# pyannote/pyannote-audio

Hardware: AMD Instinct MI355X
Metric: audio-hours/sec (real-time factor) for speaker-diarization-3.1 pipeline (higher is better)
Workload: dtype f32

## Files before the change

### include/pyannote_amd.h

```cpp
#ifndef PYANNOTE_AMD_H
#define PYANNOTE_AMD_H

#include <stddef.h>
#include <stdint.h>

#ifdef __cplusplus
extern "C" {
#endif

int pa_version(void);
const char* pa_last_error(void);

void pa_prof_enable(int on);
size_t pa_prof_report(char* buf, size_t cap);

#define PA_MAX_LSTM_LAYERS 8
#define PA_MAX_LINEAR 4

typedef struct pa_seg_weights {
  int32_t sinc_stride;
  int32_t lstm_layers;
  int32_t lstm_hidden;
  int32_t lstm_bidir;
  int32_t num_linear;
// ... 75 lines not shown
  int32_t num_blocks[4];
  int32_t planes[4];
  int32_t bottleneck;
  const float* fb_window;
  const float* fb_tw256;
  const float* fb_tw512;
  const float* fb_mel_w;
  const int32_t* fb_mel_lo;
  const int32_t* fb_mel_hi;
  const float* stem_w;
  const float* stem_shift;
  const float* blk_w1[PA_MAX_RES_BLOCKS];
  const float* blk_shift1[PA_MAX_RES_BLOCKS];
  const float* blk_w2[PA_MAX_RES_BLOCKS];
  const float* blk_shift2[PA_MAX_RES_BLOCKS];
  const float* blk_u1[PA_MAX_RES_BLOCKS];
  const float* blk_u2[PA_MAX_RES_BLOCKS];
  const float* blk_wsc[PA_MAX_RES_BLOCKS];
  const float* blk_shiftsc[PA_MAX_RES_BLOCKS];
  const float* blk_w3[PA_MAX_RES_BLOCKS];
  const float* blk_shift3[PA_MAX_RES_BLOCKS];
  const float* seg1_w;
  const float* seg1_b;
  const float* blk_v1[PA_MAX_RES_BLOCKS];
  const float* blk_v2[PA_MAX_RES_BLOCKS];
  int32_t fb_center_kernel;
} pa_emb_weights;

int pa_emb_num_fbank_frames(int num_samples);
int pa_emb_num_pool_frames(const pa_emb_weights* w, int num_samples);
size_t pa_emb_workspace_bytes(const pa_emb_weights* w, int num_chunks, int num_samples, int num_masks);
int pa_emb_forward(const pa_emb_weights* w, const float* wav, int64_t wav_len, int64_t chunk_stride,
                   int num_chunks, int num_samples, const float* masks, int num_masks, int mask_frames,
                   const int32_t* nearest_idx, float* emb, void* workspace, size_t workspace_bytes,
                   void* stream);

size_t pa_emb_ragged_workspace_bytes(const pa_emb_weights* w, int num_utterances, int max_samples);
int pa_emb_forward_ragged(const pa_emb_weights* w, const float* wav, int64_t wav_len, const int64_t* offsets,
                          const int32_t* lengths, int num_utterances, int max_samples, const float* masks, float* emb,
                          void* workspace, size_t workspace_bytes, void* stream);

size_t pa_emb_calibrate_workspace_bytes(const pa_emb_weights* w, int num_chunks, int num_samples);
int pa_emb_calibrate_winograd(const pa_emb_weights* w, const float* wav, int64_t wav_len, int64_t chunk_stride,
                              int num_chunks, int num_samples, float* report, float* emb, void* workspace,
                              size_t workspace_bytes, void* stream);
int pa_absmax_diff(const float* got, const float* ref, long n, float* out2, void* stream);

int pa_fbank(const float* wav, long wav_len, long chunk_stride, int B, int N, const float* window,
             const float* tw256, const float* tw512, const float* mel_w, const int* mel_lo,
             const int* mel_hi, int nmel, float* out, int center, void* stream);
int pa_fbank_center_span(const float* fb, int B, int T, int nmel, int kernel, float* out, void* stream);
int pa_resnet_stem(const float* fbank, int B, int T, int F, const float* w9, const float* shift,
                   float* out, void* stream);
int pa_conv3x3(const float* X, int B, int H, int W, int cin, const float* Wg, const float* shift,
               const float* R, float* Y, int cout, int stride, int relu, void* stream);
int pa_conv3x3_s2_sc_supported(int H, int cin, int cout);
int pa_conv3x3_s2_sc(const float* X, int B, int H, int W, int cin, const float* Wg, const float* shift,
                     const float* Wsc, const float* shift_sc, float* Y, float* Ysc, int cout, int relu,
                     void* stream);
int pa_winograd_pack_host(const float* conv_weight ,
                          const float* bn_scale , int cout, int cin,
                          float* U_slabs );
int pa_conv3x3_wino(const float* X, int B, int H, int W, int cin, const float* U, const float* shift,
                    const float* R, float* Y, int cout, int relu, void* stream);
int pa_winograd4_pack_host(const float* conv_weight ,
                           const float* bn_scale , int cout, int cin,
                           float* U_slabs );
int pa_conv3x3_wino4(const float* X, int B, int H, int W, int cin, const float* U, const float* shift,
                     const float* R, float* Y, int cout, int relu, void* stream);
int pa_conv3x3_wino4_rows(const float* X, int B, int H, int W, int cin, const float* U, const float* shift,
                          const float* R, float* Y, int cout, int relu, int rows, void* stream);
int pa_conv3x3_wino_rows(const float* X, int B, int H, int W, int cin, const float* U, const float* shift,
                         const float* R, float* Y, int cout, int relu, int y_first, void* stream);
int pa_stats_pool(const float* feat, int B, int Fh, int Tp, int C, const float* masks, int S, int Fm,
                  const int* nearest_idx, float* stats, void* stream);
int pa_fbank_ragged(const float* wav, long wav_len, const int64_t* offsets, const int32_t* lengths, int B,
                    int max_samples, const float* window, const float* tw256, const float* tw512, const float* mel_w,
                    const int* mel_lo, const int* mel_hi, int nmel, float* out, void* stream);
int pa_zero_tail_cols(float* x, int B, int H, int W, int C, const int32_t* lengths, int halvings, void* stream);
int pa_stats_pool_ragged(const float* feat, int B, int Fh, int W, int C, const int32_t* lengths, int halvings,
                         const float* masks, int ld_masks, float* stats, void* stream);

#define PA_W2V_MAX_CONV 8
#define PA_W2V_MAX_LAYERS 24
typedef struct pa_w2v_layer {
  const float* qk_w;
  const float* qk_b;
  const float* v_w;
  const float* out_w;
  const float* out_b;
  const float* ln1_g;
  const float* ln1_b;
  const float* ff1_w;
  const float* ff1_b;
  const float* ff2_w;
  const float* ff2_b;
  const float* ln2_g;
  const float* ln2_b;
  const float* gate_w;
  const float* gate_b;
  const float* gate_const;
} pa_w2v_layer;

typedef struct pa_sser_weights {
  int32_t num_conv;
  int32_t conv_channels[PA_W2V_MAX_CONV];
// ... 270 lines not shown
```

### pyannote-audio_amd/csrc/emb_fbank.hip

```cpp
#include "common.h"

namespace pa {

constexpr int FB_WIN = 400, FB_SHIFT = 160, FB_NFFT = 512, FB_HALF = 256, FB_NBIN = 257;
constexpr int FB_FPB = 4;

struct cplx {
  float x, y;
};
__device__ __forceinline__ cplx cmul(cplx a, cplx b) {
  return {a.x * b.x - a.y * b.y, a.x * b.y + a.y * b.x};
}

template <bool kRagged>
__global__ __launch_bounds__(256) void k_fbank(const float* __restrict__ wav, long wav_len,
                                               long chunk_stride, int T, float scale, float preemph,
                                               const float* __restrict__ window,
                                               const float2* __restrict__ tw256,
                                               const float2* __restrict__ tw512,
                                               const float* __restrict__ mel_w,
                                               const int* __restrict__ mel_lo,
                                               const int* __restrict__ mel_hi, int nmel, float eps,
                                               float* __restrict__ out, const int64_t* __restrict__ offs,
                                               const int* __restrict__ lens) {
// ... 91 lines not shown
    src = dst;
    dst = tmp;
  }
#pragma unroll
  for (int i = 0; i < 5; ++i) {
    const int k = lane + 64 * i;
    if (k <= FB_HALF) {
      const float2 zk = src[k & 255];
      const float2 zc0 = src[(FB_HALF - k) & 255];
      const cplx zc = {zc0.x, -zc0.y};
      const cplx e = {0.5f * (zk.x + zc.x), 0.5f * (zk.y + zc.y)};
      const cplx dd = {0.5f * (zk.x - zc.x), 0.5f * (zk.y - zc.y)};
      const cplx o = {dd.y, -dd.x};
      const float2 w = w512[i];
      const cplx wo = cmul(o, {w.x, w.y});
      const float re = e.x + wo.x, im = e.y + wo.y;
      xw[k] = re * re + im * im;
    }
  }
  __syncthreads();
  if (active) {
    for (int m = lane; m < nmel; m += 64) {
      const float* wrow = mel_w + (long)m * FB_NBIN;
      float acc = 0.f;
      const int lo = mel_lo[m], hi = mel_hi[m];
      for (int k0 = lo; k0 <= hi; k0 += 8) {
        float wk[8];
#pragma unroll
        for (int u = 0; u < 8; ++u) wk[u] = k0 + u <= hi ? wrow[k0 + u] : 0.f;
#pragma unroll
        for (int u = 0; u < 8; ++u)
          if (k0 + u <= hi) acc = fmaf(xw[k0 + u], wk[u], acc);
      }
      out[((long)b * T + t) * nmel + m] = logf(fmaxf(acc, eps));
    }
  }
}

__global__ __launch_bounds__(320) void k_fbank_center(float* __restrict__ fb, int T, int nmel) {
  __shared__ float part[4][80];
  const int b = blockIdx.x;
  const int m = threadIdx.x % 80, p = threadIdx.x / 80;
  float* x = fb + (long)b * T * nmel;
  float s = 0.f;
  if (m < nmel)
    for (int t = p; t < T; t += 4) s += x[(long)t * nmel + m];
  part[p][m] = s;
  __syncthreads();
  const float mean = (part[0][m] + part[1][m] + part[2][m] + part[3][m]) / (float)T;
  if (m < nmel)
    for (int t = p; t < T; t += 4) x[(long)t * nmel + m] -= mean;
}

__global__ __launch_bounds__(320) void k_fbank_center_ragged(float* __restrict__ fb, int T, int nmel,
                                                             const int* __restrict__ lens) {
  __shared__ float part[4][80];
  const int b = blockIdx.x;
  const int m = threadIdx.x % 80, p = threadIdx.x / 80;
  const int n = lens[b];
  const int Tb = n < FB_WIN ? 0 : 1 + (n - FB_WIN) / FB_SHIFT;
  float* x = fb + (long)b * T * nmel;
  float s = 0.f;
  if (m < nmel)
    for (int t = p; t < Tb; t += 4) s += x[(long)t * nmel + m];
  part[p][m] = s;
  __syncthreads();
  const float mean = (part[0][m] + part[1][m] + part[2][m] + part[3][m]) / (float)Tb;
  if (m < nmel) {
    for (int t = p; t < Tb; t += 4) x[(long)t * nmel + m] -= mean;
    for (int t = Tb + p; t < T; t += 4) x[(long)t * nmel + m] = 0.f;
  }
}

constexpr int FC_TT = 240, FC_MG = 16, FC_KMAX = 2049;
__global__ __launch_bounds__(256) void k_fbank_center_span(const float* __restrict__ fb, int T, int nmel, int K,
                                                           float* __restrict__ out) {
  extern __shared__ float fc_tile[];
  const int b = blockIdx.z, m0 = blockIdx.y * FC_MG, t0 = blockIdx.x * FC_TT;
  const int half = K >> 1;
  const int m = threadIdx.x & (FC_MG - 1), tl = threadIdx.x >> 4;
  const float* x = fb + (long)b * T * nmel;
  const int rows = FC_TT + K - 1;
  for (int r = tl; r < rows; r += 16) {
    const int t = t0 - half + r;
    fc_tile[r * FC_MG + m] = (t >= 0 && t < T && m0 + m < nmel) ? x[(long)t * nmel + m0 + m] : 0.f;
  }
  __syncthreads();
  if (m0 + m >= nmel) return;
  for (int i = tl; i < FC_TT; i += 16) {
    const int t = t0 + i;
    if (t >= T) break;
    const int lo = t - half < 0 ? 0 : t - half, hi = t + half > T - 1 ? T - 1 : t + half;
    float s = 0.f;
    for (int u = lo; u <= hi; ++u) s += fc_tile[(u - t0 + half) * FC_MG + m];
    out[((long)b * T + t) * nmel + m0 + m] = fc_tile[(i + half) * FC_MG + m] - s / (float)(hi - lo + 1);
  }
}

}

extern "C" {

int pa_fbank_center_span(const float* fb, int B, int T, int nmel, int kernel, float* out, void* stream) {
  PA_REQUIRE(kernel >= 1 && (kernel & 1), "pa_fbank_center_span: the window must be an odd number of frames (got %d)",
             kernel);
  PA_REQUIRE(fb != out, "pa_fbank_center_span: works out of place");
  if (B <= 0 || T <= 0 || nmel <= 0) return 0;
  if (kernel > 2 * T - 1) kernel = 2 * T - 1;
  PA_REQUIRE(kernel <= pa::FC_KMAX,
             "pa_fbank_center_span: a running mean over %d frames of a %d-frame chunk needs more than the LDS holds "
             "(at most %d frames)", kernel, T, pa::FC_KMAX);
  const size_t lds = (size_t)(pa::FC_TT + kernel - 1) * pa::FC_MG * sizeof(float);
  static bool attr_set = false;
  if (!attr_set) {
    (void)hipFuncSetAttribute((const void*)pa::k_fbank_center_span, hipFuncAttributeMaxDynamicSharedMemorySize,
                              (int)((pa::FC_TT + pa::FC_KMAX - 1) * pa::FC_MG * sizeof(float)));
    attr_set = true;
  }
  hipLaunchKernelGGL(pa::k_fbank_center_span, dim3(pa::cdiv(T, pa::FC_TT), pa::cdiv(nmel, pa::FC_MG), B), dim3(256), lds,
                     (hipStream_t)stream, fb, T, nmel, kernel, out);
  PA_CHECK_LAUNCH("pa_fbank_center_span");
  return 0;
}

int pa_fbank(const float* wav, long wav_len, long chunk_stride, int B, int N, const float* window,
             const float* tw256, const float* tw512, const float* mel_w, const int* mel_lo,
             const int* mel_hi, int nmel, float* out, int center, void* stream) {
  PA_REQUIRE(nmel <= 80, "pa_fbank: at most 80 mel bins are built (got %d)", nmel);
  if (B <= 0) return 0;
  PA_REQUIRE(N >= pa::FB_WIN, "pa_fbank: %d samples is shorter than one 25 ms frame", N);
  const int T = 1 + (N - pa::FB_WIN) / pa::FB_SHIFT;
  hipStream_t st = (hipStream_t)stream;
  pa::ProfScope prof("k_fbank", stream, (double)B * T * (5.0 * 512 * 9 + 2.0 * 257 * 3 + 2.0 * 257 * 2),
                     4.0 * B * N + 4.0 * B * T * nmel * (center ? 3 : 1));
  hipLaunchKernelGGL(pa::k_fbank<false>, dim3(pa::cdiv(T, pa::FB_FPB), B), dim3(256), 0, st, wav, wav_len,
                     chunk_stride, T, 32768.0f, 0.97f, window, (const float2*)tw256,
                     (const float2*)tw512, mel_w, mel_lo, mel_hi, nmel, 1.1920928955078125e-07f, out,
                     (const int64_t*)nullptr, (const int*)nullptr);
  PA_CHECK_LAUNCH("pa_fbank");
  if (center) {
    hipLaunchKernelGGL(pa::k_fbank_center, dim3(B), dim3(320), 0, st, out, T, nmel);
    PA_CHECK_LAUNCH("pa_fbank_center");
  }
  return 0;
}

int pa_fbank_ragged(const float* wav, long wav_len, const int64_t* offsets, const int32_t* lengths, int B,
                    int max_samples, const float* window, const float* tw256, const float* tw512, const float* mel_w,
                    const int* mel_lo, const int* mel_hi, int nmel, float* out, void* stream) {
  PA_REQUIRE(nmel <= 80, "pa_fbank_ragged: at most 80 mel bins are built (got %d)", nmel);
  if (B <= 0) return 0;
  PA_REQUIRE(max_samples >= pa::FB_WIN, "pa_fbank_ragged: %d samples is shorter than one 25 ms frame", max_samples);
  const int T = 1 + (max_samples - pa::FB_WIN) / pa::FB_SHIFT;
  hipStream_t st = (hipStream_t)stream;
  pa::ProfScope prof("k_fbank_ragged", stream, (double)B * T * (5.0 * 512 * 9 + 2.0 * 257 * 3 + 2.0 * 257 * 2),
                     4.0 * B * max_samples + 12.0 * B * T * nmel);
  hipLaunchKernelGGL(pa::k_fbank<true>, dim3(pa::cdiv(T, pa::FB_FPB), B), dim3(256), 0, st, wav, wav_len, 0L, T,
                     32768.0f, 0.97f, window, (const float2*)tw256, (const float2*)tw512, mel_w, mel_lo, mel_hi, nmel,
                     1.1920928955078125e-07f, out, offsets, (const int*)lengths);
  PA_CHECK_LAUNCH("pa_fbank_ragged");
  hipLaunchKernelGGL(pa::k_fbank_center_ragged, dim3(B), dim3(320), 0, st, out, T, nmel, (const int*)lengths);
  PA_CHECK_LAUNCH("pa_fbank_center_ragged");
  return 0;
}

}
```

### pyannote-audio_amd/csrc/emb_forward.cpp

```cpp
#include "forward_common.h"

namespace {

struct EmbPlan {
  int B, N, T, F, S;
  int Hs[5], Ws[5];
  size_t fbank, act[4], stats, total, act_elems;
  size_t t2_off, gather_off;
};

inline bool s2_fold_wanted() {
  static const bool fold = getenv("PA_S2_FOLD") == nullptr || atoi(getenv("PA_S2_FOLD")) != 0;
  return fold;
}

inline bool prefer_wino4(int H, int W, int cin) {
  auto up = [](int a, int b) { return (long)((a + b - 1) / b) * b; };
  long p4 = up(H, 4) * up(W, 64);
  const long p4_lin = up(H, 4) * up(W, 4);
  if (p4_lin * 120 <= p4 * 100) p4 = p4_lin * 120 / 100;
  long p2 = up(H, 8) * up(W, 32);
  if (up(H, 4) * up(W, 64) < p2) p2 = up(H, 4) * up(W, 64);
  if (up(H, 2) * up(W, 128) < p2) p2 = up(H, 2) * up(W, 128);
  const long gain = cin >= 256 ? 130 : 122;
  return p4 * 100 <= p2 * gain;
}

bool make_plan(const pa_emb_weights* w, int B, int N, int S, EmbPlan* p, bool calib = false) {
  if (N < 400) return false;
  p->B = B;
  p->N = N;
  p->S = S < 1 ? 1 : S;
  p->T = 1 + (N - 400) / 160;
  p->F = w->num_mel;
  p->Hs[0] = p->F;
  p->Ws[0] = p->T;
  for (int l = 0; l < w->num_layers; ++l) {
    const int s = l == 0 ? 1 : 2;
    p->Hs[l + 1] = (p->Hs[l] - 1) / s + 1;
    p->Ws[l + 1] = (p->Ws[l] - 1) / s + 1;
  }
  pa::Bump ws;
  p->fbank = ws.take((size_t)B * p->T * p->F);
  const int ex = w->bottleneck ? 4 : 1;
  p->act_elems = (size_t)B * p->Hs[0] * p->Ws[0] * w->planes[0] * ex;
  for (int i = 0; i < 3; ++i) p->act[i] = ws.take(p->act_elems);
  p->t2_off = p->gather_off = 0;
  if (w->bottleneck) {
    size_t t1 = 0, t2 = 0, g = 0;
    int cin = w->planes[0];
    for (int l = 0; l < w->num_layers; ++l) {
      const size_t planes = w->planes[l];
      const size_t in_px = (size_t)B * p->Hs[l == 0 ? 1 : l] * p->Ws[l == 0 ? 1 : l];
      const size_t out_px = (size_t)B * p->Hs[l + 1] * p->Ws[l + 1];
      t1 = t1 > in_px * planes ? t1 : in_px * planes;
      t2 = t2 > out_px * planes ? t2 : out_px * planes;
      if (l > 0) g = g > out_px * cin ? g : out_px * cin;
      cin = 4 * (int)planes;
    }
    p->t2_off = pa::Bump::align(t1);
    p->gather_off = p->t2_off + pa::Bump::align(t2);
    p->act[3] = ws.take(p->gather_off + pa::Bump::align(g));
  } else if (calib) {
    p->act[3] = ws.take(p->act_elems);
  }
  const int L = w->num_layers;
// ... 1 lines not shown
  p->total = ws.o;
  return true;
}

}

extern "C" {

int pa_emb_num_fbank_frames(int num_samples) {
  return num_samples < 400 ? 0 : 1 + (num_samples - 400) / 160;
}

int pa_emb_num_pool_frames(const pa_emb_weights* w, int num_samples) {
  EmbPlan p;
  if (!make_plan(w, 1, num_samples, 1, &p)) return 0;
  return p.Ws[w->num_layers];
}

size_t pa_emb_workspace_bytes(const pa_emb_weights* w, int num_chunks, int num_samples, int num_masks) {
  EmbPlan p;
  if (!make_plan(w, num_chunks, num_samples, num_masks, &p)) return 0;
  return p.total * sizeof(float);
}

}


static int emb_forward_impl(const pa_emb_weights* w, const float* wav, int64_t wav_len, int64_t chunk_stride,
                            int num_chunks, int num_samples, const float* masks, int num_masks, int mask_frames,
                            const int32_t* nearest_idx, float* emb, void* workspace, size_t workspace_bytes,
                            void* stream, float* calib, const int64_t* offsets = nullptr,
                            const int32_t* lengths = nullptr) {
  if (num_chunks <= 0) return 0;
  const bool ragged = lengths != nullptr;
  EmbPlan p;
  if (w->num_layers != 4 || !make_plan(w, num_chunks, num_samples, masks ? num_masks : 1, &p, calib != nullptr)) {
    pa::set_error("pa_emb_forward: %d samples is too short (fbank needs >= 400) or bad layer count",
                  num_samples);
    return 3;
  }
  if (workspace_bytes < p.total * sizeof(float)) {
    pa::set_error("pa_emb_forward: workspace too small (%zu < %zu bytes)", workspace_bytes,
                  p.total * sizeof(float));
    return 3;
  }
  float* ws = (float*)workspace;
  const int B = p.B;

  const int span = w->fb_center_kernel;
  if (ragged && span != 0) {
    pa::set_error("pa_emb_forward_ragged: fbank_centering_span checkpoints run one launch sequence per length");
    return 3;
  }
  if (ragged)
    PA_RUN(pa_fbank_ragged(wav, wav_len, offsets, lengths, B, p.N, w->fb_window, w->fb_tw256, w->fb_tw512, w->fb_mel_w,
                           w->fb_mel_lo, w->fb_mel_hi, w->num_mel, ws + p.fbank, stream));
  else
    PA_RUN(pa_fbank(wav, wav_len, chunk_stride, B, p.N, w->fb_window, w->fb_tw256, w->fb_tw512, w->fb_mel_w,
                    w->fb_mel_lo, w->fb_mel_hi, w->num_mel, ws + p.fbank, span == 0 ? 1 : 0, stream));
  auto zero_tail = [&](float* X, int l, int C) -> int {
    return ragged ? pa_zero_tail_cols(X, B, p.Hs[l], p.Ws[l], C, lengths, l > 0 ? l - 1 : 0, stream) : 0;
  };
  float* cur = ws + p.act[0];
  float* f1 = ws + p.act[1];
  float* f2 = ws + p.act[2];
  const float* feats = ws + p.fbank;
  if (span != 0) {
    PA_RUN(pa_fbank_center_span(ws + p.fbank, B, p.T, p.F, span, f1, stream));
    feats = f1;
  }
  PA_RUN(pa_resnet_stem(feats, B, p.T, p.F, w->stem_w, w->stem_shift, cur, stream));
  if (!w->bottleneck) PA_RUN(zero_tail(cur, 0, w->planes[0]));

  auto conv_s1 = [&](const float* X, int H, int W, int ci, const float* v, const float* u, const float* wd,
                     const float* shift, const float* R, float* Y, int co, int slot) -> int {
    if (calib != nullptr) {
      float* scratch = ws + p.act[3];
      float* rep = calib + 4 * slot;
      const long n = (long)B * H * W * co;
      int r = pa_conv3x3(X, B, H, W, ci, wd, shift, R, Y, co, 1, 1, stream);
      if (r == 0 && v != nullptr) {
        r = pa_conv3x3_wino4(X, B, H, W, ci, v, shift, R, scratch, co, 1, stream);
        if (r == 0) r = pa_absmax_diff(scratch, Y, n, rep, stream);
      }
      if (r == 0 && u != nullptr) {
        r = pa_conv3x3_wino(X, B, H, W, ci, u, shift, R, scratch, co, 1, stream);
        if (r == 0) r = pa_absmax_diff(scratch, Y, n, rep + 2, stream);
      }
      return r;
    }
    if (v != nullptr && prefer_wino4(H, W, ci)) return pa_conv3x3_wino4(X, B, H, W, ci, v, shift, R, Y, co, 1, stream);
    if (u != nullptr) return pa_conv3x3_wino(X, B, H, W, ci, u, shift, R, Y, co, 1, stream);
    return pa_conv3x3(X, B, H, W, ci, wd, shift, R, Y, co, 1, 1, stream);
  };

  int blk = 0;
  int cin = w->planes[0];
  if (w->bottleneck) {
    float* nxt = f1;
    float* sc = f2;
    float* tmp = ws + p.act[3];
    for (int l = 0; l < w->num_layers; ++l) {
      const int planes = w->planes[l], cout = 4 * planes;
      for (int i = 0; i < w->num_blocks[l]; ++i, ++blk) {
        if (blk >= PA_MAX_RES_BLOCKS) {
          pa::set_error("pa_emb_forward: more than %d residual blocks", PA_MAX_RES_BLOCKS);
          return 3;
        }
        const int stride = (i == 0 && l > 0) ? 2 : 1;
        const int H = stride == 2 ? p.Hs[l] : p.Hs[l + 1], W = stride == 2 ? p.Ws[l] : p.Ws[l + 1];
        const int Ho = p.Hs[l + 1], Wo = p.Ws[l + 1];
        float* t1 = tmp;
        float* t2 = tmp + p.t2_off;
        PA_RUN(pa_gemm_tn_ex(cur, cin, w->blk_w1[blk], cin, w->blk_shift1[blk], nullptr, t1, planes, B * H * W,
                             planes, cin, 2, 0, stream));
        PA_RUN(zero_tail(t1, stride == 2 ? l : l + 1, planes));
        if (stride == 1 && w->blk_u2[blk] != nullptr)
          PA_RUN(pa_conv3x3_wino(t1, B, H, W, planes, w->blk_u2[blk], w->blk_shift2[blk], nullptr, t2, planes, 1,
                                 stream));
        else
          PA_RUN(pa_conv3x3(t1, B, H, W, planes, w->blk_w2[blk], w->blk_shift2[blk], nullptr, t2, planes, stride,
                            1, stream));
        const float* res = cur;
        if (w->blk_wsc[blk] != nullptr) {
// ... 127 lines not shown
```

### pyannote-audio_amd/csrc/emb_resnet.hip

```cpp
#include "common.h"

namespace pa {

constexpr int STEM_TS = 64;
constexpr int STEM_LD = STEM_TS + 3;

__global__ __launch_bounds__(256) void k_stem(const float* __restrict__ fb, int T, int F,
                                              const float* __restrict__ w9,
                                              const float* __restrict__ shift,
                                              float* __restrict__ out) {
  extern __shared__ float xs[];
  const int b = blockIdx.y, t0 = blockIdx.x * STEM_TS;
  const int tid = threadIdx.x;
  for (int i = tid; i < 2 * STEM_LD; i += 256) xs[(i < STEM_LD ? 0 : (F + 1) * STEM_LD - STEM_LD) + i] = 0.f;
  const int n = (STEM_TS + 2) * F;
  for (int i0 = 0; i0 < n; i0 += 8 * 256) {
    float v[8];
#pragma unroll
    for (int k = 0; k < 8; ++k) {
      const int i = i0 + tid + 256 * k;
      const int tt = i / F, ff = i - tt * F, t = t0 + tt - 1;
      v[k] = (i < n && t >= 0 && t < T) ? fb[((long)b * T + t) * F + ff] : 0.f;
    }
#pragma unroll
    for (int k = 0; k < 8; ++k) {
      const int i = i0 + tid + 256 * k;
      const int tt = i / F, ff = i - tt * F;
      if (i < n) xs[(ff + 1) * STEM_LD + tt] = v[k];
    }
  }
  const int q4 = (tid & 7) * 4, pl = tid >> 3;
  float w[9][4], sh[4];
#pragma unroll
  for (int k = 0; k < 9; ++k)
#pragma unroll
    for (int c = 0; c < 4; ++c) w[k][c] = w9[k * 32 + q4 + c];
#pragma unroll
  for (int c = 0; c < 4; ++c) sh[c] = shift[q4 + c];
  __syncthreads();
  float x0[2][3], x1[2][3], x2[2][3];
#pragma unroll
  for (int h = 0; h < 2; ++h)
#pragma unroll
    for (int dt = 0; dt < 3; ++dt) {
      x0[h][dt] = xs[0 * STEM_LD + pl + 32 * h + dt];
      x1[h][dt] = xs[1 * STEM_LD + pl + 32 * h + dt];
    }
  const bool ok0 = t0 + pl < T, ok1 = t0 + pl + 32 < T;
  float* o = out + ((long)b * F * T + t0 + pl) * 32 + q4;
  for (int f = 0; f < F; ++f) {
#pragma unroll
    for (int h = 0; h < 2; ++h)
#pragma unroll
      for (int dt = 0; dt < 3; ++dt) x2[h][dt] = xs[(f + 2) * STEM_LD + pl + 32 * h + dt];
    float* of = o + (long)f * T * 32;
#pragma unroll
    for (int h = 0; h < 2; ++h) {
      float acc[4];
#pragma unroll
      for (int c = 0; c < 4; ++c) acc[c] = 0.f;
#pragma unroll
      for (int dt = 0; dt < 3; ++dt)
#pragma unroll
        for (int c = 0; c < 4; ++c) acc[c] = fmaf(x0[h][dt], w[dt][c], acc[c]);
#pragma unroll
      for (int dt = 0; dt < 3; ++dt)
#pragma unroll
        for (int c = 0; c < 4; ++c) acc[c] = fmaf(x1[h][dt], w[3 + dt][c], acc[c]);
#pragma unroll
      for (int dt = 0; dt < 3; ++dt)
#pragma unroll
        for (int c = 0; c < 4; ++c) acc[c] = fmaf(x2[h][dt], w[6 + dt][c], acc[c]);
      float4 o4;
      o4.x = fmaxf(acc[0] + sh[0], 0.f);
      o4.y = fmaxf(acc[1] + sh[1], 0.f);
// ... 263 lines not shown
                         hipStream_t st) {
  using G = ConvGeom<TH, TWT>;
  const int Ho = H, Wo = W;
  const int tiles_w = cdiv(Wo, G::TW), tiles_h = cdiv(Ho, TH);
  const size_t lds = (size_t)(G::PATCH + 9 * BN * CLD) * sizeof(float);
  constexpr int MAXDEV = 16;
  static int resident_of[MAXDEV] = {0}, per_cu_of[MAXDEV] = {0};
  int dev = 0;
  (void)hipGetDevice(&dev);
  if (dev < 0 || dev >= MAXDEV) dev = 0;
  if (!resident_of[dev]) {
    (void)hipFuncSetAttribute((const void*)k_conv3x3<TH, TWT, BN, HAS_R>,
                              hipFuncAttributeMaxDynamicSharedMemorySize, (int)lds);
    int cus = 256, per_cu = 2;
    (void)hipDeviceGetAttribute(&cus, hipDeviceAttributeMultiprocessorCount, dev);
    if (hipOccupancyMaxActiveBlocksPerMultiprocessor(&per_cu, k_conv3x3<TH, TWT, BN, HAS_R>, 256, lds) !=
            hipSuccess || per_cu < 1)
      per_cu = 2;
    resident_of[dev] = cus * per_cu;
    per_cu_of[dev] = per_cu;
  }
  const int resident = resident_of[dev] & ~7;
  const int tiles_hw = tiles_w * tiles_h, n_tiles = COUT / BN;
  const long total = (long)tiles_hw * n_tiles * B;
  const int grid = (int)(total < resident ? total : resident);
  int* counters = tile_counters();
  if (counters == nullptr) {
    set_error("pa_conv3x3: cannot allocate the tile counters");
    return 2;
  }
  hipLaunchKernelGGL((k_conv3x3<TH, TWT, BN, HAS_R>), dim3(grid), dim3(256), lds, st, X, H, W, CIN, Wg,
                     shift, R, Y, Ho, Wo, COUT, relu, tiles_w, tiles_hw, n_tiles, (int)total, xcd_ranges_wanted(true),
                     counters);
  return 0;
}

template <int TH, int TWT, int BN>
static int launch_conv(const float* X, int B, int H, int W, int CIN, const float* Wg,
                       const float* shift, const float* R, float* Y, int COUT, int relu,
                       hipStream_t st) {
  return R != nullptr ? launch_conv_r<TH, TWT, BN, true>(X, B, H, W, CIN, Wg, shift, R, Y, COUT, relu, st)
                      : launch_conv_r<TH, TWT, BN, false>(X, B, H, W, CIN, Wg, shift, R, Y, COUT, relu, st);
}

}

extern "C" {

int pa_resnet_stem(const float* fbank, int B, int T, int F, const float* w9, const float* shift,
                   float* out, void* stream) {
  if (B <= 0) return 0;
  pa::ProfScope prof("k_stem", stream, 2.0 * B * T * F * 9 * 32, 4.0 * B * T * F * 33);
  PA_REQUIRE(F >= 1 && (size_t)(F + 2) * pa::STEM_LD * 4 <= 64 * 1024, "pa_resnet_stem: %d mel bins do not fit LDS", F);
  hipLaunchKernelGGL(pa::k_stem, dim3(pa::cdiv(T, pa::STEM_TS), B), dim3(256), (size_t)(F + 2) * pa::STEM_LD * 4,
                     (hipStream_t)stream, fbank, T, F, w9, shift, out);
  PA_CHECK_LAUNCH("pa_resnet_stem");
  return 0;
}

int pa_conv3x3(const float* X, int B, int H, int W, int cin, const float* Wg, const float* shift,
               const float* R, float* Y, int cout, int stride, int relu, void* stream) {
  if (B <= 0) return 0;
  PA_REQUIRE(cin % pa::CB == 0 && cout % 32 == 0, "pa_conv3x3: cin %% 16 and cout %% 32 required");
  hipStream_t st = (hipStream_t)stream;
  const int Ho = (H - 1) / stride + 1, Wo_ = (W - 1) / stride + 1;
  pa::ProfScope prof("k_conv3x3", stream, 2.0 * 9 * cin * cout * (double)B * Ho * Wo_,
                     4.0 * ((double)B * H * W * cin + (double)B * Ho * Wo_ * cout * (R ? 2 : 1) + 9.0 * cin * cout));
  if (stride == 1) {
    if (cout == 32) pa::launch_conv<8, 1, 32>(X, B, H, W, cin, Wg, shift, R, Y, cout, relu, st);
    else if (Ho >= 32) pa::launch_conv<8, 1, 64>(X, B, H, W, cin, Wg, shift, R, Y, cout, relu, st);
    else if (Ho >= 16) pa::launch_conv<4, 2, 64>(X, B, H, W, cin, Wg, shift, R, Y, cout, relu, st);
    else pa::launch_conv<2, 2, 64>(X, B, H, W, cin, Wg, shift, R, Y, cout, relu, st);
  } else if (stride == 2) {
    PA_REQUIRE(cout % 64 == 0, "pa_conv3x3: stride 2 needs cout %% 64 == 0");
    if (pa::launch_conv_s2(X, B, H, W, cin, Wg, shift, R, Y, cout, relu, st) != 0) return 2;
  } else {
    PA_REQUIRE(false, "pa_conv3x3: stride %d not supported", stride);
  }
  PA_CHECK_LAUNCH("pa_conv3x3");
  return 0;
}

int pa_conv3x3_s2_sc_supported(int H, int cin, int cout) {
  return H >= 1 && cin >= pa::CB && cin % pa::CB == 0 && cout >= 64 && cout % 64 == 0 && (H - 1) / 2 + 1 >= 16;
}

int pa_conv3x3_s2_sc(const float* X, int B, int H, int W, int cin, const float* Wg, const float* shift,
                     const float* Wsc, const float* shift_sc, float* Y, float* Ysc, int cout, int relu,
                     void* stream) {
  if (B <= 0) return 0;
  PA_REQUIRE(cin >= pa::CB && cin % pa::CB == 0, "pa_conv3x3_s2_sc: cin %% 16 == 0 required");
  PA_REQUIRE(cout >= 64 && cout % 64 == 0, "pa_conv3x3_s2_sc: cout %% 64 == 0 required");
  const int Ho = (H - 1) / 2 + 1, Wo_ = (W - 1) / 2 + 1;
  PA_REQUIRE(H >= 1 && W >= 1 && Ho >= 16, "pa_conv3x3_s2_sc: at least 16 output rows required (got %d)", Ho);
  const size_t n_out = (size_t)B * Ho * Wo_ * cout;
  PA_REQUIRE(Y != nullptr && Ysc != nullptr && (Y + n_out <= Ysc || Ysc + n_out <= Y),
             "pa_conv3x3_s2_sc: Y and Ysc overlap");
  pa::ProfScope prof("k_conv3x3", stream, 2.0 * (9 + 1) * cin * cout * (double)B * Ho * Wo_,
                     4.0 * ((double)B * H * W * cin + 2.0 * (double)B * Ho * Wo_ * cout + 10.0 * cin * cout));
  if (pa::launch_conv_s2_sc(X, B, H, W, cin, Wg, shift, Wsc, shift_sc, Y, Ysc, cout, relu, (hipStream_t)stream) != 0)
    return 2;
  PA_CHECK_LAUNCH("pa_conv3x3_s2_sc");
  return 0;
}

}
```

### pyannote-audio_amd/ffi.py

```python
from __future__ import annotations

import ctypes as C
from pathlib import Path

import torch

_LIB = None
PA_MAX_LSTM_LAYERS = 8
PA_MAX_LINEAR = 4

c_fp = C.c_void_p


class SegWeights(C.Structure):
    _fields_ = [
        ("sinc_stride", C.c_int32), ("lstm_layers", C.c_int32), ("lstm_hidden", C.c_int32),
        ("lstm_bidir", C.c_int32), ("num_linear", C.c_int32), ("linear_hidden", C.c_int32),
        ("num_classes", C.c_int32), ("num_speakers", C.c_int32),
        ("wav_gamma", C.c_float), ("wav_beta", C.c_float),
        ("sinc_filt", c_fp), ("norm0", c_fp), ("conv1_w", c_fp), ("conv1_b", c_fp), ("norm1", c_fp),
        ("conv2_w", c_fp), ("conv2_b", c_fp), ("norm2", c_fp),
        ("lstm_wih", c_fp * PA_MAX_LSTM_LAYERS), ("lstm_bias", c_fp * PA_MAX_LSTM_LAYERS),
        ("lstm_whh", c_fp * PA_MAX_LSTM_LAYERS),
        ("lin_w", c_fp * PA_MAX_LINEAR), ("lin_b", c_fp * PA_MAX_LINEAR),
# ... 123 lines not shown
                                     C.c_float, C.c_float, c_fp, c_fp, c_fp]
    lib.pa_sinc_fir_span.argtypes = [c_fp, C.c_long, C.c_long, c_fp, c_fp, c_fp]
    lib.pa_sinc_fix_pool.argtypes = [c_fp, C.c_long, C.c_int, C.c_int, C.c_int, c_fp, c_fp, C.c_float, C.c_float,
                                     c_fp, c_fp, c_fp, c_fp]
    lib.pa_sinc_fir_span_centred.argtypes = [c_fp, C.c_long, C.c_long, c_fp, c_fp, c_fp, c_fp, c_fp]
    lib.pa_sinc_fix_pool_centred.argtypes = [c_fp, C.c_long, C.c_int, C.c_int, C.c_int, c_fp, C.c_long, C.c_int, c_fp,
                                             c_fp, C.c_float, C.c_float, c_fp, c_fp, c_fp, c_fp]
    lib.pa_conv5_pool.argtypes = [c_fp, C.c_int, C.c_int, C.c_int, c_fp, c_fp, c_fp, c_fp, c_fp, c_fp,
                                  c_fp, c_fp]
    lib.pa_norm_transpose.argtypes = [c_fp, C.c_int, C.c_int, c_fp, c_fp, c_fp, c_fp, c_fp, c_fp]
    lib.pa_gemm_tn_ex.argtypes = [c_fp, C.c_int, c_fp, C.c_int, c_fp, c_fp, c_fp, C.c_long, C.c_int, C.c_int,
                                  C.c_int, C.c_int, C.c_int, c_fp]
    lib.pa_gemm_tn.argtypes = [c_fp, C.c_int, c_fp, C.c_int, c_fp, c_fp, C.c_long, C.c_int, C.c_int,
                               C.c_int, C.c_int, C.c_int, c_fp]
    lib.pa_lstm_rec.argtypes = [c_fp, c_fp, c_fp, C.c_int, C.c_int, C.c_int, c_fp]
    lib.pa_classifier.argtypes = [c_fp, C.c_int, C.c_int, C.c_int, C.c_int, C.c_int, c_fp, c_fp,
                                  C.c_int, c_fp, C.c_int, c_fp, c_fp, c_fp]
    lib.pa_prof_enable.argtypes = [C.c_int]
    lib.pa_prof_enable.restype = None
    lib.pa_prof_report.argtypes = [C.c_char_p, C.c_size_t]
    lib.pa_prof_report.restype = C.c_size_t
    _declare_optional(lib)
    _LIB = lib
    return lib


_OPTIONAL: list[tuple] = [
    ("pa_emb_num_fbank_frames", [C.c_int], C.c_int),
    ("pa_emb_num_pool_frames", [C.POINTER(EmbWeights), C.c_int], C.c_int),
    ("pa_emb_workspace_bytes", [C.POINTER(EmbWeights), C.c_int, C.c_int, C.c_int], C.c_size_t),
    ("pa_emb_forward", [C.POINTER(EmbWeights), c_fp, C.c_int64, C.c_int64, C.c_int, C.c_int, c_fp,
                        C.c_int, C.c_int, c_fp, c_fp, c_fp, C.c_size_t, c_fp], C.c_int),
    ("pa_emb_ragged_workspace_bytes", [C.POINTER(EmbWeights), C.c_int, C.c_int], C.c_size_t),
    ("pa_emb_forward_ragged", [C.POINTER(EmbWeights), c_fp, C.c_int64, c_fp, c_fp, C.c_int, C.c_int, c_fp, c_fp,
                               c_fp, C.c_size_t, c_fp], C.c_int),
    ("pa_fbank_ragged", [c_fp, C.c_long, c_fp, c_fp, C.c_int, C.c_int, c_fp, c_fp, c_fp, c_fp, c_fp, c_fp, C.c_int,
                         c_fp, c_fp], C.c_int),
    ("pa_zero_tail_cols", [c_fp, C.c_int, C.c_int, C.c_int, C.c_int, c_fp, C.c_int, c_fp], C.c_int),
    ("pa_stats_pool_ragged", [c_fp, C.c_int, C.c_int, C.c_int, C.c_int, c_fp, C.c_int, c_fp, C.c_int, c_fp, c_fp],
     C.c_int),
    ("pa_emb_calibrate_workspace_bytes", [C.POINTER(EmbWeights), C.c_int, C.c_int], C.c_size_t),
    ("pa_emb_calibrate_winograd", [C.POINTER(EmbWeights), c_fp, C.c_int64, C.c_int64, C.c_int, C.c_int, c_fp, c_fp,
                                   c_fp, C.c_size_t, c_fp], C.c_int),
    ("pa_lstm_rec_h", [c_fp, c_fp, c_fp, C.c_int, C.c_int, C.c_int, C.c_int, c_fp], C.c_int),
    ("pa_absmax_diff", [c_fp, c_fp, C.c_long, c_fp, c_fp], C.c_int),
    ("pa_gemm_tn_s2", [c_fp, C.c_int, C.c_int, C.c_int, C.c_int, c_fp, C.c_int, c_fp, c_fp, C.c_long, C.c_int,
                       c_fp], C.c_int),
    ("pa_gemm_tn_batched", [c_fp, C.c_int, C.c_long, C.c_long, c_fp, C.c_int, C.c_long, C.c_long, c_fp, c_fp, C.c_long,
                            C.c_long, C.c_long, C.c_int, C.c_int, C.c_int, C.c_int, C.c_int, C.c_int, c_fp], C.c_int),
    ("pa_fbank", [c_fp, C.c_long, C.c_long, C.c_int, C.c_int, c_fp, c_fp, c_fp, c_fp, c_fp, c_fp,
                  C.c_int, c_fp, C.c_int, c_fp], C.c_int),
    ("pa_fbank_center_span", [c_fp, C.c_int, C.c_int, C.c_int, C.c_int, c_fp, c_fp], C.c_int),
    ("pa_resnet_stem", [c_fp, C.c_int, C.c_int, C.c_int, c_fp, c_fp, c_fp, c_fp], C.c_int),
    ("pa_conv3x3", [c_fp, C.c_int, C.c_int, C.c_int, C.c_int, c_fp, c_fp, c_fp, c_fp, C.c_int, C.c_int,
                    C.c_int, c_fp], C.c_int),
    ("pa_conv3x3_s2_sc_supported", [C.c_int, C.c_int, C.c_int], C.c_int),
    ("pa_conv3x3_s2_sc", [c_fp, C.c_int, C.c_int, C.c_int, C.c_int, c_fp, c_fp, c_fp, c_fp, c_fp, c_fp, C.c_int,
                          C.c_int, c_fp], C.c_int),
    ("pa_conv3x3_wino", [c_fp, C.c_int, C.c_int, C.c_int, C.c_int, c_fp, c_fp, c_fp, c_fp, C.c_int, C.c_int,
                         c_fp], C.c_int),
    ("pa_conv3x3_wino4", [c_fp, C.c_int, C.c_int, C.c_int, C.c_int, c_fp, c_fp, c_fp, c_fp, C.c_int, C.c_int,
                          c_fp], C.c_int),
    ("pa_conv3x3_wino4_rows", [c_fp, C.c_int, C.c_int, C.c_int, C.c_int, c_fp, c_fp, c_fp, c_fp, C.c_int, C.c_int,
                               C.c_int, c_fp], C.c_int),
    ("pa_conv3x3_wino_rows", [c_fp, C.c_int, C.c_int, C.c_int, C.c_int, c_fp, c_fp, c_fp, c_fp, C.c_int, C.c_int,
                              C.c_int, c_fp], C.c_int),
    ("pa_pdist_f64", [c_fp, C.c_int, C.c_int, c_fp, c_fp], C.c_int),
    ("pa_cdist_cosine_f64", [c_fp, C.c_int, c_fp, C.c_int, C.c_int, c_fp, c_fp, c_fp], C.c_int),
    ("pa_centroid_means", [c_fp, C.c_int, c_fp, c_fp, C.c_int, c_fp, c_fp], C.c_int),
    ("pa_linkage_workspace_bytes", [C.c_int], C.c_size_t),
    ("pa_linkage_centroid_f64", [c_fp, C.c_int, c_fp, c_fp, C.c_size_t, c_fp], C.c_int),
    ("pa_linkage_centroid_f64_ex", [c_fp, C.c_int, c_fp, c_fp, C.c_size_t, C.c_int, c_fp], C.c_int),
    ("pa_pdist_cosine_f64", [c_fp, C.c_int, C.c_int, c_fp, c_fp, c_fp], C.c_int),
    ("pa_nonfinite_flag_f64", [c_fp, C.c_long, c_fp, c_fp], C.c_int),
    ("pa_linkage_chain_workspace_bytes", [C.c_int], C.c_size_t),
    ("pa_linkage_chain_f64", [c_fp, C.c_int, C.c_int, c_fp, c_fp, C.c_size_t, c_fp], C.c_int),
    ("pa_seg_files_workspace_bytes", [C.POINTER(SegWeights), C.c_int, c_fp, C.c_int, C.c_int64], C.c_size_t),
    ("pa_seg_forward_files", [C.POINTER(SegWeights), c_fp, c_fp, c_fp, C.c_int, C.c_int64, C.c_int, c_fp, c_fp, c_fp,
                              C.c_size_t, c_fp], C.c_int),
    ("pa_gather_chunks", [c_fp, c_fp, c_fp, c_fp, C.c_int, C.c_int, c_fp, c_fp], C.c_int),
    ("pa_seg_chunk_stats", [c_fp, C.c_int, C.c_int, C.c_int, c_fp, c_fp, c_fp], C.c_int),
    ("pa_embedding_masks", [c_fp, C.c_int, C.c_int, C.c_int, c_fp, C.c_int, C.c_int, c_fp, c_fp], C.c_int),
    ("pa_speaker_count", [c_fp, C.c_int, C.c_int, C.c_int, c_fp, C.c_int, c_fp, c_fp, c_fp], C.c_int),
    ("pa_cluster_activations", [c_fp, C.c_int, C.c_int, C.c_int, c_fp, c_fp, C.c_int, C.c_int, c_fp, c_fp],
     C.c_int),
    ("pa_topk_binarize", [c_fp, c_fp, C.c_int, C.c_int, C.c_int, c_fp, c_fp, c_fp], C.c_int),
    ("pa_topk_binarize_f32", [c_fp, c_fp, C.c_int, C.c_int, C.c_int, c_fp, c_fp, c_fp], C.c_int),
    ("pa_binarize_hysteresis", [c_fp, C.c_int, C.c_int, C.c_int, C.c_float, C.c_float, C.c_int, c_fp, c_fp],
     C.c_int),
    ("pa_cluster_max", [c_fp, C.c_int, C.c_int, C.c_int, c_fp, C.c_int, c_fp, c_fp], C.c_int),
    ("pa_aggregate", [c_fp, C.c_int, C.c_int, C.c_int, c_fp, C.c_int, c_fp, c_fp, C.c_float, C.c_float, C.c_int,
                      c_fp, c_fp], C.c_int),
    ("pa_binarize_regions_workspace_bytes", [C.c_int, C.c_int, C.c_int], C.c_size_t),
    ("pa_binarize_regions", [c_fp, C.c_int, C.c_int, c_fp, c_fp, c_fp, c_fp, C.c_double, C.c_double, C.c_double,
                             C.c_int, c_fp, c_fp, c_fp, c_fp, C.c_size_t, c_fp], C.c_int),
    ("pa_regions_sweep_groups", [C.c_int, C.c_int, c_fp], C.c_int),
    ("pa_regions_sweep_workspace_bytes", [C.c_int, C.c_int, C.c_int, C.c_int, C.c_int, C.c_long, C.c_long],
     C.c_size_t),
    ("pa_regions_sweep_count", [c_fp, C.c_int, C.c_int, C.c_int, c_fp, c_fp, c_fp, c_fp, c_fp, c_fp, C.c_size_t,
                                c_fp], C.c_int),
    ("pa_regions_sweep_emit", [c_fp, C.c_int, C.c_int, C.c_int, c_fp, c_fp, c_fp, c_fp, C.c_int, c_fp, c_fp, c_fp,
                               C.c_double, C.c_double, C.c_double, C.c_long, c_fp, c_fp, c_fp, c_fp, c_fp, C.c_size_t,
                               c_fp], C.c_int),
    ("pa_resample_poly", [c_fp, C.c_long, c_fp, C.c_int, C.c_int, C.c_int, C.c_int, c_fp, C.c_long, c_fp],
     C.c_int),
    ("pa_plda_transform", [c_fp, C.c_int, C.c_int, C.c_int, C.c_int, c_fp, c_fp, c_fp, c_fp, c_fp, c_fp, c_fp],
# ... 129 lines not shown
```

Measured before the change: 1.345.

## Compute fbank frames once across overlapping chunks and center inside stem

When chunks overlap with a stride that is a multiple of the 160-sample hop, the filterbank is computed once over the whole shared frame sequence instead of once per chunk. Per-chunk means are taken in a small kernel, and the stem conv subtracts the mean while loading. This removes the redundant FFT/mel work on overlapping frames and the in-place centering pass, at the cost of an extra mean kernel and a subtraction per stem load. It can be disabled through an environment variable.

```diff
diff --git a/include/pyannote_amd.h b/include/pyannote_amd.h
--- a/include/pyannote_amd.h
+++ b/include/pyannote_amd.h
@@ -151,6 +151,12 @@
 int pa_fbank_center_span(const float* fb, int B, int T, int nmel, int kernel, float* out, void* stream);
 int pa_resnet_stem(const float* fbank, int B, int T, int F, const float* w9, const float* shift,
                    float* out, void* stream);
+int pa_fbank_frames(const float* wav, long wav_len, long num_frames, const float* window, const float* tw256,
+                    const float* tw512, const float* mel_w, const int* mel_lo, const int* mel_hi, int nmel, float* out,
+                    void* stream);
+int pa_fbank_chunk_means(const float* frames, int B, int T, int chunk_rows, int nmel, float* mean, void* stream);
+int pa_resnet_stem_shared(const float* frames, const float* mean, int B, int T, int F, int chunk_rows, const float* w9,
+                          const float* shift, float* out, void* stream);
 int pa_conv3x3(const float* X, int B, int H, int W, int cin, const float* Wg, const float* shift,
                const float* R, float* Y, int cout, int stride, int relu, void* stream);
 int pa_conv3x3_s2_sc_supported(int H, int cin, int cout);
diff --git a/pyannote-audio_amd/csrc/emb_fbank.hip b/pyannote-audio_amd/csrc/emb_fbank.hip
--- a/pyannote-audio_amd/csrc/emb_fbank.hip
+++ b/pyannote-audio_amd/csrc/emb_fbank.hip
@@ -167,6 +167,20 @@
     for (int t = p; t < T; t += 4) x[(long)t * nmel + m] -= mean;
 }
 
+__global__ __launch_bounds__(320) void k_fbank_chunk_mean(const float* __restrict__ frames, int T, int chunk_rows,
+                                                          int nmel, float* __restrict__ mean) {
+  __shared__ float part[4][80];
+  const int b = blockIdx.x;
+  const int m = threadIdx.x % 80, p = threadIdx.x / 80;
+  const float* x = frames + (long)b * chunk_rows * nmel;
+  float s = 0.f;
+  if (m < nmel)
+    for (int t = p; t < T; t += 4) s += x[(long)t * nmel + m];
+  part[p][m] = s;
+  __syncthreads();
+  if (p == 0 && m < nmel) mean[(long)b * nmel + m] = (part[0][m] + part[1][m] + part[2][m] + part[3][m]) / (float)T;
+}
+
 __global__ __launch_bounds__(320) void k_fbank_center_ragged(float* __restrict__ fb, int T, int nmel,
                                                              const int* __restrict__ lens) {
   __shared__ float part[4][80];
@@ -260,6 +274,35 @@
   return 0;
 }
 
+int pa_fbank_frames(const float* wav, long wav_len, long num_frames, const float* window, const float* tw256,
+                    const float* tw512, const float* mel_w, const int* mel_lo, const int* mel_hi, int nmel, float* out,
+                    void* stream) {
+  PA_REQUIRE(nmel <= 80, "pa_fbank_frames: at most 80 mel bins are built (got %d)", nmel);
+  if (num_frames <= 0) return 0;
+  PA_REQUIRE(num_frames <= 0x7fffffffL - pa::FB_FPB, "pa_fbank_frames: %ld frames are more than one launch takes",
+             num_frames);
+  const int T = (int)num_frames;
+  const double samples = (double)(num_frames - 1) * pa::FB_SHIFT + pa::FB_WIN;
+  pa::ProfScope prof("k_fbank", stream, (double)T * (5.0 * 512 * 9 + 2.0 * 257 * 3 + 2.0 * 257 * 2),
+                     4.0 * samples + 4.0 * T * nmel);
+  hipLaunchKernelGGL(pa::k_fbank<false>, dim3(pa::cdiv(T, pa::FB_FPB), 1), dim3(256), 0, (hipStream_t)stream, wav,
+                     wav_len, 0L, T, 32768.0f, 0.97f, window, (const float2*)tw256, (const float2*)tw512, mel_w, mel_lo,
+                     mel_hi, nmel, 1.1920928955078125e-07f, out, (const int64_t*)nullptr, (const int*)nullptr);
+  PA_CHECK_LAUNCH("pa_fbank_frames");
+  return 0;
+}
+
+int pa_fbank_chunk_means(const float* frames, int B, int T, int chunk_rows, int nmel, float* mean, void* stream) {
+  PA_REQUIRE(nmel <= 80, "pa_fbank_chunk_means: at most 80 mel bins are built (got %d)", nmel);
+  PA_REQUIRE(T >= 1 && chunk_rows >= 0, "pa_fbank_chunk_means: %d frames per chunk, %d rows apart", T, chunk_rows);
+  if (B <= 0) return 0;
+  pa::ProfScope prof("k_fbank_chunk_mean", stream, (double)B * T * nmel, 4.0 * B * T * nmel + 4.0 * B * nmel);
+  hipLaunchKernelGGL(pa::k_fbank_chunk_mean, dim3(B), dim3(320), 0, (hipStream_t)stream, frames, T, chunk_rows, nmel,
+                     mean);
+  PA_CHECK_LAUNCH("pa_fbank_chunk_means");
+  return 0;
+}
+
 int pa_fbank_ragged(const float* wav, long wav_len, const int64_t* offsets, const int32_t* lengths, int B,
                     int max_samples, const float* window, const float* tw256, const float* tw512, const float* mel_w,
                     const int* mel_lo, const int* mel_hi, int nmel, float* out, void* stream) {
diff --git a/pyannote-audio_amd/csrc/emb_fbank_plan.h b/pyannote-audio_amd/csrc/emb_fbank_plan.h
--- /dev/null
+++ b/pyannote-audio_amd/csrc/emb_fbank_plan.h
@@ -0,0 +1,28 @@
+#pragma once
+
+namespace pa {
+
+constexpr int FBP_WIN = 400, FBP_HOP = 160;
+
+struct FbankSharedPlan {
+  bool shared;
+  int T;
+  int chunk_rows;
+  long frames;
+};
+
+inline int fbank_chunk_frames(int N) { return N < FBP_WIN ? 0 : 1 + (N - FBP_WIN) / FBP_HOP; }
+
+inline FbankSharedPlan fbank_shared_plan(bool ragged, int center_kernel, int B, int N, long stride) {
+  FbankSharedPlan p;
+  p.T = fbank_chunk_frames(N);
+  p.shared = !ragged && center_kernel == 0 && B >= 2 && p.T > 0 && stride >= 0 && stride % FBP_HOP == 0 &&
+             stride / FBP_HOP < p.T;
+  p.chunk_rows = p.shared ? (int)(stride / FBP_HOP) : 0;
+  p.frames = p.shared ? (long)(B - 1) * p.chunk_rows + p.T : (long)(B > 0 ? B : 0) * p.T;
+  return p;
+}
+
+inline long fbank_shared_row(const FbankSharedPlan& p, int b, int t) { return (long)b * p.chunk_rows + t; }
+
+}
diff --git a/pyannote-audio_amd/csrc/emb_forward.cpp b/pyannote-audio_amd/csrc/emb_forward.cpp
--- a/pyannote-audio_amd/csrc/emb_forward.cpp
+++ b/pyannote-audio_amd/csrc/emb_forward.cpp
@@ -1,4 +1,5 @@
 #include "forward_common.h"
+#include "emb_fbank_plan.h"
 
 namespace {
 
@@ -12,6 +13,11 @@
 inline bool s2_fold_wanted() {
   static const bool fold = getenv("PA_S2_FOLD") == nullptr || atoi(getenv("PA_S2_FOLD")) != 0;
   return fold;
+}
+
+inline bool fbank_shared_wanted() {
+  static const bool shared = getenv("PA_FBANK_SHARED") == nullptr || atoi(getenv("PA_FBANK_SHARED")) != 0;
+  return shared;
 }
 
 inline bool prefer_wino4(int H, int W, int cin) {
@@ -119,7 +125,12 @@
     pa::set_error("pa_emb_forward_ragged: fbank_centering_span checkpoints run one launch sequence per length");
     return 3;
   }
-  if (ragged)
+  pa::FbankSharedPlan fp = pa::fbank_shared_plan(ragged, span, B, p.N, chunk_stride);
+  if (!fbank_shared_wanted()) fp.shared = false;
+  if (fp.shared)
+    PA_RUN(pa_fbank_frames(wav, wav_len, fp.frames, w->fb_window, w->fb_tw256, w->fb_tw512, w->fb_mel_w, w->fb_mel_lo,
+                           w->fb_mel_hi, w->num_mel, ws + p.fbank, stream));
+  else if (ragged)
     PA_RUN(pa_fbank_ragged(wav, wav_len, offsets, lengths, B, p.N, w->fb_window, w->fb_tw256, w->fb_tw512, w->fb_mel_w,
                            w->fb_mel_lo, w->fb_mel_hi, w->num_mel, ws + p.fbank, stream));
   else
@@ -136,7 +147,11 @@
     PA_RUN(pa_fbank_center_span(ws + p.fbank, B, p.T, p.F, span, f1, stream));
     feats = f1;
   }
-  PA_RUN(pa_resnet_stem(feats, B, p.T, p.F, w->stem_w, w->stem_shift, cur, stream));
+  if (fp.shared) {
+    PA_RUN(pa_fbank_chunk_means(feats, B, p.T, fp.chunk_rows, p.F, f1, stream));
+    PA_RUN(pa_resnet_stem_shared(feats, f1, B, p.T, p.F, fp.chunk_rows, w->stem_w, w->stem_shift, cur, stream));
+  } else
+    PA_RUN(pa_resnet_stem(feats, B, p.T, p.F, w->stem_w, w->stem_shift, cur, stream));
   if (!w->bottleneck) PA_RUN(zero_tail(cur, 0, w->planes[0]));
 
   auto conv_s1 = [&](const float* X, int H, int W, int ci, const float* v, const float* u, const float* wd,
diff --git a/pyannote-audio_amd/csrc/emb_resnet.hip b/pyannote-audio_amd/csrc/emb_resnet.hip
--- a/pyannote-audio_amd/csrc/emb_resnet.hip
+++ b/pyannote-audio_amd/csrc/emb_resnet.hip
@@ -5,22 +5,29 @@
 constexpr int STEM_TS = 64;
 constexpr int STEM_LD = STEM_TS + 3;
 
+template <bool kShared>
 __global__ __launch_bounds__(256) void k_stem(const float* __restrict__ fb, int T, int F,
                                               const float* __restrict__ w9,
                                               const float* __restrict__ shift,
-                                              float* __restrict__ out) {
+                                              float* __restrict__ out, const float* __restrict__ mean,
+                                              int chunk_rows) {
   extern __shared__ float xs[];
   const int b = blockIdx.y, t0 = blockIdx.x * STEM_TS;
   const int tid = threadIdx.x;
   for (int i = tid; i < 2 * STEM_LD; i += 256) xs[(i < STEM_LD ? 0 : (F + 1) * STEM_LD - STEM_LD) + i] = 0.f;
   const int n = (STEM_TS + 2) * F;
+  const float* fbb = fb + (long)b * (kShared ? chunk_rows : T) * F;
   for (int i0 = 0; i0 < n; i0 += 8 * 256) {
     float v[8];
 #pragma unroll
     for (int k = 0; k < 8; ++k) {
       const int i = i0 + tid + 256 * k;
       const int tt = i / F, ff = i - tt * F, t = t0 + tt - 1;
-      v[k] = (i < n && t >= 0 && t < T) ? fb[((long)b * T + t) * F + ff] : 0.f;
+      const bool in = i < n && t >= 0 && t < T;
+      if constexpr (kShared)
+        v[k] = in ? fbb[(long)t * F + ff] - mean[(long)b * F + ff] : 0.f;
+      else
+        v[k] = in ? fbb[(long)t * F + ff] : 0.f;
     }
 #pragma unroll
     for (int k = 0; k < 8; ++k) {
@@ -390,9 +397,23 @@
   if (B <= 0) return 0;
   pa::ProfScope prof("k_stem", stream, 2.0 * B * T * F * 9 * 32, 4.0 * B * T * F * 33);
   PA_REQUIRE(F >= 1 && (size_t)(F + 2) * pa::STEM_LD * 4 <= 64 * 1024, "pa_resnet_stem: %d mel bins do not fit LDS", F);
-  hipLaunchKernelGGL(pa::k_stem, dim3(pa::cdiv(T, pa::STEM_TS), B), dim3(256), (size_t)(F + 2) * pa::STEM_LD * 4,
-                     (hipStream_t)stream, fbank, T, F, w9, shift, out);
+  hipLaunchKernelGGL(pa::k_stem<false>, dim3(pa::cdiv(T, pa::STEM_TS), B), dim3(256), (size_t)(F + 2) * pa::STEM_LD * 4,
+                     (hipStream_t)stream, fbank, T, F, w9, shift, out, (const float*)nullptr, 0);
   PA_CHECK_LAUNCH("pa_resnet_stem");
+  return 0;
+}
+
+int pa_resnet_stem_shared(const float* frames, const float* mean, int B, int T, int F, int chunk_rows, const float* w9,
+                          const float* shift, float* out, void* stream) {
+  if (B <= 0) return 0;
+  pa::ProfScope prof("k_stem", stream, 2.0 * B * T * F * 9 * 32,
+                     4.0 * B * T * F * 32 + 4.0 * ((double)(B - 1) * chunk_rows + T) * F + 4.0 * B * F);
+  PA_REQUIRE(F >= 1 && (size_t)(F + 2) * pa::STEM_LD * 4 <= 64 * 1024, "pa_resnet_stem_shared: %d mel bins do not fit LDS",
+             F);
+  PA_REQUIRE(T >= 1 && chunk_rows >= 0, "pa_resnet_stem_shared: %d frames per chunk, %d rows apart", T, chunk_rows);
+  hipLaunchKernelGGL(pa::k_stem<true>, dim3(pa::cdiv(T, pa::STEM_TS), B), dim3(256), (size_t)(F + 2) * pa::STEM_LD * 4,
+                     (hipStream_t)stream, frames, T, F, w9, shift, out, mean, chunk_rows);
+  PA_CHECK_LAUNCH("pa_resnet_stem_shared");
   return 0;
 }
 
diff --git a/pyannote-audio_amd/ffi.py b/pyannote-audio_amd/ffi.py
--- a/pyannote-audio_amd/ffi.py
+++ b/pyannote-audio_amd/ffi.py
@@ -199,6 +199,9 @@
                   C.c_int, c_fp, C.c_int, c_fp], C.c_int),
     ("pa_fbank_center_span", [c_fp, C.c_int, C.c_int, C.c_int, C.c_int, c_fp, c_fp], C.c_int),
     ("pa_resnet_stem", [c_fp, C.c_int, C.c_int, C.c_int, c_fp, c_fp, c_fp, c_fp], C.c_int),
+    ("pa_fbank_frames", [c_fp, C.c_long, C.c_long, c_fp, c_fp, c_fp, c_fp, c_fp, c_fp, C.c_int, c_fp, c_fp], C.c_int),
+    ("pa_fbank_chunk_means", [c_fp, C.c_int, C.c_int, C.c_int, C.c_int, c_fp, c_fp], C.c_int),
+    ("pa_resnet_stem_shared", [c_fp, c_fp, C.c_int, C.c_int, C.c_int, C.c_int, c_fp, c_fp, c_fp, c_fp], C.c_int),
     ("pa_conv3x3", [c_fp, C.c_int, C.c_int, C.c_int, C.c_int, c_fp, c_fp, c_fp, c_fp, C.c_int, C.c_int,
                     C.c_int, c_fp], C.c_int),
     ("pa_conv3x3_s2_sc_supported", [C.c_int, C.c_int, C.c_int], C.c_int),
```

Result: no change. 1.356, median of 6 (+0.8%).
